# bennyguo/instant-nsr-pl

Measured on NVIDIA H100. Metric: rays/sec fwd+bwd (NeRF-Synthetic lego shape), higher is better.
Workload: dtype f16

## Files before the change

### instant-nsr-pl_b200/csrc/nerf_fused_bwd.cu

```cuda
#include "nerf_fused.cuh"
#include "wgmma.cuh"

namespace {

constexpr int kWarps = 4;
constexpr int kThreads = kWarps * 32;
constexpr int kRows = kWarps * 16;
constexpr int kCtasPerSm = 2;

constexpr int T_X0 = 0;
constexpr int T_H1 = T_X0 + kRows * NF_LD32;
constexpr int T_CI = T_H1 + kRows * NSR_LD64;
constexpr int T_G1 = T_CI + kRows * NF_LD32;
constexpr int T_G2 = T_G1 + kRows * NSR_LD64;
constexpr int T_DC3 = T_G2 + kRows * NSR_LD64;
constexpr int T_DG2 = T_DC3 + kRows * 24;
constexpr int T_DG1 = T_DG2 + kRows * NSR_LD64;
constexpr int T_DO = T_DG1 + kRows * NSR_LD64;
constexpr int T_DH1 = T_DO + kRows * 24;
constexpr int T_X0B = T_DH1 + kRows * NSR_LD64;
constexpr int T_TOTAL = T_X0B + kRows * NF_LD32;
constexpr int S_XYZ = 0, S_DS = S_XYZ + kRows * 6, S_DRGB = S_DS + kRows, S_ROWF = S_DRGB + kRows * 3;
constexpr size_t kSmemBytes = (size_t)(NF_W_TOTAL + T_TOTAL) * sizeof(__half) + 2 * S_ROWF * sizeof(float);
constexpr size_t kSmemBytesVanilla = kSmemBytes + NF_B_TOTAL * sizeof(float);
// ... 191 lines not shown
            for (int e = 0; e < 2; ++e) {
              const int col = c * 2 + e;
              if (col < 3) {
                const float raw = NET == NF_NET_VANILLA ? acc16[0][0][hh * 2 + e] : __half2float(__float2half_rn(acc16[0][0][hh * 2 + e]));
                const float s = 1.f / (1.f + expf(-raw));
                const float dr = PACKED ? rf[S_DRGB + (r0 + g + hh * 8) * 3 + col] : d_rgb[pi * 3 + col];
                dp[hh * 2 + e] = dr * s * (1.f - s) * loss_scale;
              }
            }
          }
        }
      }
      a_dc3[0][0][0] = nsr_pack_h2(dp[0], dp[1]);
      a_dc3[0][0][1] = nsr_pack_h2(dp[2], dp[3]);
      a_dc3[0][0][2] = 0u;
      a_dc3[0][0][3] = 0u;
      nsr_store_afrag<1, 1>(a_dc3, T + T_DC3, 24, r0);
    }
    uint32_t a_d[1][4][4];
    nsr_zero_acc(acc);
    nsr_gemm_wt<1, 1, 8>(acc, a_dc3, smem + NF_OFF_CW3, NSR_LD64);
    relu_mask_pack(acc, a_g2, a_d);
    nsr_store_afrag<1, 4>(a_d, T + T_DG2, NSR_LD64, r0);
    nsr_zero_acc(acc);
    nsr_gemm_wt<1, 4, 8>(acc, a_d, smem + NF_OFF_CW2, NSR_LD64);
    relu_mask_pack(acc, a_g1, a_d);
    nsr_store_afrag<1, 4>(a_d, T + T_DG1, NSR_LD64, r0);
    nsr_zero_acc(acc16);
    nsr_gemm_wt<1, 4, 2>(acc16, a_d, smem + NF_OFF_CW1, NF_LD32);
    if (c == 0) {
      if (ia < n) acc16[0][0][0] += (PACKED ? rf[S_DS + r0 + g] : d_sraw[pa]) * loss_scale;
      if (ib < n) acc16[0][0][2] += (PACKED ? rf[S_DS + r0 + g + 8] : d_sraw[pb]) * loss_scale;
    }
    uint32_t a_do[1][1][4];
    nsr_acc_to_afrag<1, 2>(acc16, a_do, NSR_ACT_NONE);
    nsr_store_afrag<1, 1>(a_do, T + T_DO, 24, r0);
    nsr_zero_acc(acc);
    nsr_gemm_wt<1, 1, 8>(acc, a_do, smem + NF_OFF_DW2, NSR_LD64);
    relu_mask_pack(acc, a_h1, a_d);
    nsr_store_afrag<1, 4>(a_d, T + T_DH1, NSR_LD64, r0);
    float accE[1][4][4];
    nsr_zero_acc(accE);
    nsr_gemm_wt<1, 4, 4>(accE, a_d, smem + NF_OFF_DW1, NF_LD32);

#pragma unroll
    for (int hh = 0; hh < 2; ++hh) {
      const int64_t i = hh ? ib : ia;
      const bool ok = i < n;
      float x = 0.f, y = 0.f, z = 0.f, dx, dy, dz;
      if (ok) {
        if (PACKED) {
          const float* rr = rf + S_XYZ + (r0 + g + hh * 8) * 6;
          x = rr[0];
          y = rr[1];
          z = rr[2];
        } else {
          nf_sample_position<CT>(P, rays, ray_indices[i], t_starts[i], t_ends[i], x, y, z, dx, dy, dz);
        }
      }
#pragma unroll
      for (int nt = 0; nt < 4; ++nt) {
        const float d0 = ok ? accE[0][nt][hh * 2] * inv_scale : 0.f, d1 = ok ? accE[0][nt][hh * 2 + 1] * inv_scale : 0.f;
        const LevelInfo li = nsr_level(P.grid, nt * 4 + c);
        uint32_t cx, cy, cz, idx[8];
        float fx, fy, fz;
        nsr_pos_fract(x, li.scale, cx, fx);
        nsr_pos_fract(y, li.scale, cy, fy);
        nsr_pos_fract(z, li.scale, cz, fz);
        if (nt < 2) {
          const uint32_t key = ok ? (cx + li.res * (cy + li.res * cz)) : (0xFFFFFFF0u + g);
          const uint32_t key_prev = __shfl_up_sync(0xffffffffu, key, 4);
          const bool head = (g == 0) || (key_prev != key);
          const int next_head = __shfl_down_sync(0xffffffffu, (int)head, 4);
          const bool tail = (g == 7) || next_head;
          float v[16];
#pragma unroll
          for (int cc = 0; cc < 8; ++cc) {
            const float w = nsr_corner_weight(cc, fx, fy, fz);
            v[2 * cc] = w * d0;
            v[2 * cc + 1] = w * d1;
          }
          bool flag = head;
#pragma unroll
          for (int o = 1; o < 8; o <<= 1) {
            const int f_up = __shfl_up_sync(0xffffffffu, (int)flag, 4 * o);
            const bool take = (g >= o) && !flag;
#pragma unroll
            for (int e = 0; e < 16; ++e) {
              const float u = __shfl_up_sync(0xffffffffu, v[e], 4 * o);
              if (take) v[e] += u;
            }
            if (take) flag = f_up;
          }
          if (ok && tail) {
            nsr_corner_indices(li, cx, cy, cz, idx);
#pragma unroll
            for (int cc = 0; cc < 8; ++cc)
              if (v[2 * cc] != 0.f || v[2 * cc + 1] != 0.f) nsr_red_add_f32x2(grad_table + 2 * (size_t)idx[cc], v[2 * cc], v[2 * cc + 1]);
          }
        } else if (ok && (d0 != 0.f || d1 != 0.f)) {
          nsr_corner_indices(li, cx, cy, cz, idx);
#pragma unroll
          for (int cc = 0; cc < 8; ++cc) {
            const float w = nsr_corner_weight(cc, fx, fy, fz);
            nsr_red_add_f32x2(grad_table + 2 * (size_t)idx[cc], w * d0, w * d1);
          }
        }
      }
    }
    __syncthreads();
#pragma unroll
    for (int s = 0; s < kSlots; ++s) {
      const WgradTile w = wgrad_tile(warp + s * kWarps);
      const int xo = (w.x_off == T_X0) ? x0_off : w.x_off;
      nsr_wgrad_tile(wacc[s][0], wacc[s][1], T + w.dy_off, w.ldy, w.m0, T + xo, w.ldx, w.n0, kRows);
    }
    if (NET == NF_NET_VANILLA) {
#pragma unroll
      for (int q = 0; q < 2; ++q) {
        const int j = threadIdx.x + q * kThreads;
        if (j < NF_B_TOTAL) {
          const __half* col = j < NF_B_D2 ? T + T_DH1 + j : j < NF_B_C1 ? T + T_DO + (j - NF_B_D2) : j < NF_B_C2 ? T + T_DG1 + (j - NF_B_C1)
                                                                                      : j < NF_B_C3 ? T + T_DG2 + (j - NF_B_C2) : T + T_DC3 + (j - NF_B_C3);
          const int ld = (j >= NF_B_D2 && j < NF_B_C1) || j >= NF_B_C3 ? 24 : NSR_LD64;
          float sum = 0.f;
#pragma unroll 8
          for (int r = 0; r < kRows; ++r) sum += __half2float(col[r * ld]);
          bsum[q] += sum;
        }
      }
    }
  }
  if (NET == NF_NET_VANILLA) {
#pragma unroll
    for (int q = 0; q < 2; ++q) {
      const int j = threadIdx.x + q * kThreads;
      if (j < NF_B_TOTAL && bsum[q] != 0.f) atomicAdd(j < NF_B_C1 ? grad_dbias + j : grad_cbias + (j - NF_B_C1), bsum[q] * inv_scale);
    }
  }
#pragma unroll
  for (int s = 0; s < kSlots; ++s) {
    const WgradTile w = wgrad_tile(warp + s * kWarps);
    float* dst = (w.net == 0 ? grad_dparams : grad_cparams) + w.base;
#pragma unroll
    for (int j = 0; j < 2; ++j)
#pragma unroll
      for (int i = 0; i < 4; ++i) {
        const int o = w.m0 + g + ((i >> 1) << 3), ii = w.n0 + j * 8 + c * 2 + (i & 1);
        atomicAdd(dst + (size_t)o * w.in_dim + ii, wacc[s][j][i] * inv_scale);
      }
  }
}

constexpr int kNetThreads = 384;
constexpr int SL_X0 = 0;
constexpr int SL_CI = SL_X0 + kRows * 32 * 2;
constexpr int SL_H1 = SL_CI + kRows * 32 * 2;
constexpr int SL_G1 = SL_H1 + kRows * 64 * 2;
constexpr int SL_G2 = SL_G1 + kRows * 64 * 2;
constexpr int SL_DC3 = SL_G2 + kRows * 64 * 2;
constexpr int SL_DO = SL_DC3 + kRows * 16 * 2;
constexpr int SL_DG2 = SL_DO + kRows * 16 * 2;
constexpr int SL_DG1 = SL_DG2 + kRows * 64 * 2;
constexpr int SL_DH1 = SL_DG1 + kRows * 64 * 2;
constexpr int kSlotBytes = SL_DH1 + kRows * 64 * 2;
constexpr int kNetSlots = 3;
constexpr int N_SLOTS = NF_W_TOTAL * 2;
constexpr int N_STAGE = N_SLOTS + kNetSlots * kSlotBytes;
constexpr int kStageBytes = kRows * NF_LD32 * 2 + S_ROWF * 4;
constexpr int N_BARS = N_STAGE + 2 * kStageBytes;
constexpr size_t kNetSmemBytes = N_BARS + 2 * kNetSlots * 8;
static_assert(N_SLOTS % 128 == 0 && kSlotBytes % 128 == 0 && kStageBytes % 16 == 0 && N_BARS % 8 == 0, "alignment");
static_assert(kNetSmemBytes <= 227 * 1024, "shared memory");

template <int KT>
__device__ __forceinline__ void canon_load_afrag(uint32_t (&a)[1][KT][4], const uint8_t* tile, int K, int row0, int col0 = 0) {
  const int lane = threadIdx.x & 31, mi = lane >> 3, r = lane & 7;
#pragma unroll
  for (int k = 0; k < KT; ++k) nsr_ldmatrix_x4(a[0][k], tile + nsr_canon_off(row0 + (mi & 1) * 8 + r, col0 + k * 16 + (mi >> 1) * 8, K));
}
template <int KT>
__device__ __forceinline__ void canon_store_afrag(const uint32_t (&a)[1][KT][4], uint8_t* tile, int K, int row0, int col0 = 0) {
  const int lane = threadIdx.x & 31, g = lane >> 2, c = lane & 3;
#pragma unroll
  for (int k = 0; k < KT; ++k) {
    const int col = col0 + k * 16 + c * 2;
    *reinterpret_cast<uint32_t*>(tile + nsr_canon_off(row0 + g, col, K)) = a[0][k][0];
    *reinterpret_cast<uint32_t*>(tile + nsr_canon_off(row0 + g + 8, col, K)) = a[0][k][1];
    *reinterpret_cast<uint32_t*>(tile + nsr_canon_off(row0 + g, col + 8, K)) = a[0][k][2];
    *reinterpret_cast<uint32_t*>(tile + nsr_canon_off(row0 + g + 8, col + 8, K)) = a[0][k][3];
  }
}
__device__ __forceinline__ void group_bar(int grp) { asm volatile("bar.sync %0, 128;" ::"r"(1 + grp) : "memory"); }

template <int R>
__device__ __forceinline__ void net_flush(const float (&w)[R], float* dst, int stride_m, int stride_n, float inv_scale) {
  const int lane = threadIdx.x & 31, m0 = 16 * ((threadIdx.x >> 5) & 3) + (lane >> 2), c0 = 2 * (lane & 3);
#pragma unroll
  for (int r = 0; r < R; ++r) {
    const int j = r >> 2, h = (r >> 1) & 1, e = r & 1;
    atomicAdd(dst + (size_t)(m0 + 8 * h) * stride_m + (size_t)(8 * j + c0 + e) * stride_n, w[r] * inv_scale);
  }
}

__global__ void __launch_bounds__(kNetThreads, 1) nerf_bwd_net_kernel(const __half* __restrict__ enc_save, const __half* __restrict__ dparams,
                                                                      const __half* __restrict__ cparams, const float* __restrict__ d_sraw,
                                                                      const float* __restrict__ d_rgb, float* __restrict__ grad_dparams,
                                                                      float* __restrict__ grad_cparams, float loss_scale,
                                                                      const float* __restrict__ amax_ptr, int64_t n_cap,
                                                                      const int64_t* __restrict__ n_dev, const float* __restrict__ xyzdir,
                                                                      uint32_t* __restrict__ denc_out) {
  const int64_t n = n_dev ? min(*n_dev, n_cap) : n_cap;
  extern __shared__ __align__(128) uint8_t smem_net[];
  __half* W = reinterpret_cast<__half*>(smem_net);
  const int warp = threadIdx.x >> 5, lane = threadIdx.x & 31;
  if (loss_scale <= 0.f) {
    const float amax = fmaxf(__ldg(amax_ptr), 1e-30f);
    loss_scale = exp2f(fminf(fmaxf(floorf(log2f(256.f / amax)), -24.f), 60.f));
  }
  const float inv_scale = 1.f / loss_scale;
  const uint32_t sbase = nsr_smem_u32(smem_net);
  auto full_bar = [&](int s) { return sbase + N_BARS + 8u * (uint32_t)s; };
  auto empty_bar = [&](int s) { return sbase + N_BARS + 8u * (uint32_t)(kNetSlots + s); };
  if (threadIdx.x == 0) {
    for (int s = 0; s < kNetSlots; ++s) {
      mbar_init(full_bar(s), 128);
      mbar_init(empty_bar(s), 128);
    }
    asm volatile("fence.mbarrier_init.release.cluster;" ::: "memory");
  }
  nf_stage_weights(W, dparams, cparams, true);
  __syncthreads();
  const int64_t n_tiles = (n + kRows - 1) / kRows;
  const int64_t my_tiles = n_tiles > (int64_t)blockIdx.x ? (n_tiles - 1 - blockIdx.x) / gridDim.x + 1 : 0;

  if (warp < 8) {
    const int grp = warp >> 2, gtid = threadIdx.x & 127, g = lane >> 2, c = lane & 3;
    const int r0 = (warp & 3) * 16;
    __half* sx = reinterpret_cast<__half*>(smem_net + N_STAGE + grp * kStageBytes);
    float* rf = reinterpret_cast<float*>(smem_net + N_STAGE + grp * kStageBytes + kRows * NF_LD32 * 2);
    auto fetch_tile = [&](int64_t it) {
      const int64_t row0 = ((int64_t)blockIdx.x + it * gridDim.x) * kRows;
      for (int v = gtid; v < kRows * 4; v += 128) cp_async16(sx + (v >> 2) * NF_LD32 + (v & 3) * 8, enc_save + (row0 + (v >> 2)) * 32 + (v & 3) * 8);
      if (gtid < kRows * 6 / 4) cp_async16(rf + S_XYZ + gtid * 4, xyzdir + row0 * 6 + gtid * 4);
      if (gtid < kRows / 4) cp_async16(rf + S_DS + gtid * 4, d_sraw + row0 + gtid * 4);
      if (gtid >= 64 && gtid < 64 + kRows * 3 / 4) cp_async16(rf + S_DRGB + (gtid - 64) * 4, d_rgb + row0 * 3 + (gtid - 64) * 4);
      cp_async_commit();
    };
    if (grp < my_tiles) fetch_tile(grp);
    for (int64_t it = grp; it < my_tiles; it += 2) {
      const int s = (int)(it % kNetSlots);
      const int64_t row0 = ((int64_t)blockIdx.x + it * gridDim.x) * kRows;
      cp_async_wait_all();
      group_bar(grp);
      if (row0 + kRows > n) {
        for (int v = gtid; v < kRows * 4; v += 128)
          if (row0 + (v >> 2) >= n) *reinterpret_cast<uint4*>(sx + (v >> 2) * NF_LD32 + (v & 3) * 8) = make_uint4(0, 0, 0, 0);
        for (int v = gtid; v < S_ROWF; v += 128) {
          const int r = v < S_DS ? v / 6 : (v < S_DRGB ? v - S_DS : (v - S_DRGB) / 3);
          if (row0 + r >= n) rf[v] = 0.f;
        }
        group_bar(grp);
      }
      if (it >= kNetSlots) mbar_wait(empty_bar(s), (uint32_t)((it / kNetSlots - 1) & 1), nullptr, 0);
      uint8_t* slot = smem_net + N_SLOTS + s * kSlotBytes;
      const int64_t ia = row0 + r0 + g, ib = ia + 8;
      uint32_t a_in[1][2][4];
      nsr_load_afrag<1, 2>(a_in, sx, NF_LD32, r0);
      canon_store_afrag<2>(a_in, slot + SL_X0, 32, r0);
      if (lane < 16) {
        uint4 s0 = make_uint4(0, 0, 0, 0), s1 = s0;
        if (row0 + r0 + lane < n) {
          float sh[16];
          const float* rr = rf + S_XYZ + (r0 + lane) * 6;
          nsr_sh4(rr[3], rr[4], rr[5], sh);
          s0 = make_uint4(nsr_pack_h2(sh[0], sh[1]), nsr_pack_h2(sh[2], sh[3]), nsr_pack_h2(sh[4], sh[5]), nsr_pack_h2(sh[6], sh[7]));
          s1 = make_uint4(nsr_pack_h2(sh[8], sh[9]), nsr_pack_h2(sh[10], sh[11]), nsr_pack_h2(sh[12], sh[13]), nsr_pack_h2(sh[14], sh[15]));
        }
        *reinterpret_cast<uint4*>(slot + SL_CI + nsr_canon_off(r0 + lane, 16, 32)) = s0;
        *reinterpret_cast<uint4*>(slot + SL_CI + nsr_canon_off(r0 + lane, 24, 32)) = s1;
      }
      float drgb[2][2], dsr[2];
#pragma unroll
      for (int hh = 0; hh < 2; ++hh) {
#pragma unroll
        for (int e = 0; e < 2; ++e) drgb[hh][e] = (c * 2 + e < 3) ? rf[S_DRGB + (r0 + g + hh * 8) * 3 + c * 2 + e] : 0.f;
        dsr[hh] = rf[S_DS + r0 + g + hh * 8];
      }
      group_bar(grp);
      if (it + 2 < my_tiles) fetch_tile(it + 2);

      uint32_t a_h1[1][4][4], a_o[1][1][4], a_g1[1][4][4], a_g2[1][4][4];
      float acc[1][8][4], acc16[1][2][4];
      nsr_zero_acc(acc);
      nsr_gemm_w<1, 2, 8>(acc, a_in, W + NF_OFF_DW1, NF_LD32);
      nsr_acc_to_afrag<1, 8>(acc, a_h1, NSR_ACT_RELU);
      canon_store_afrag<4>(a_h1, slot + SL_H1, 64, r0);
      nsr_zero_acc(acc16);
      nsr_gemm_w<1, 4, 2>(acc16, a_h1, W + NF_OFF_DW2, NSR_LD64);
      nsr_acc_to_afrag<1, 2>(acc16, a_o, NSR_ACT_NONE);
      canon_store_afrag<1>(a_o, slot + SL_CI, 32, r0);
      __syncwarp();
      {
        uint32_t a_c[1][2][4], a_sh[1][1][4];
        canon_load_afrag<1>(a_sh, slot + SL_CI, 32, r0, 16);
#pragma unroll
        for (int j = 0; j < 4; ++j) {
          a_c[0][0][j] = a_o[0][0][j];
          a_c[0][1][j] = a_sh[0][0][j];
        }
        nsr_zero_acc(acc);
        nsr_gemm_w<1, 2, 8>(acc, a_c, W + NF_OFF_CW1, NF_LD32);
      }
      nsr_acc_to_afrag<1, 8>(acc, a_g1, NSR_ACT_RELU);
      canon_store_afrag<4>(a_g1, slot + SL_G1, 64, r0);
      nsr_zero_acc(acc);
      nsr_gemm_w<1, 4, 8>(acc, a_g1, W + NF_OFF_CW2, NSR_LD64);
      nsr_acc_to_afrag<1, 8>(acc, a_g2, NSR_ACT_RELU);
      canon_store_afrag<4>(a_g2, slot + SL_G2, 64, r0);
      nsr_zero_acc(acc16);
      nsr_gemm_w<1, 4, 2>(acc16, a_g2, W + NF_OFF_CW3, NSR_LD64);
      uint32_t a_dc3[1][1][4];
      {
        float dp[4] = {0.f, 0.f, 0.f, 0.f};
        if (c < 2) {
#pragma unroll
          for (int hh = 0; hh < 2; ++hh) {
            if ((hh ? ib : ia) < n) {
#pragma unroll
              for (int e = 0; e < 2; ++e) {
                if (c * 2 + e < 3) {
                  const float raw = __half2float(__float2half_rn(acc16[0][0][hh * 2 + e]));
                  const float sg = 1.f / (1.f + expf(-raw));
                  dp[hh * 2 + e] = drgb[hh][e] * sg * (1.f - sg) * loss_scale;
                }
              }
            }
          }
        }
        a_dc3[0][0][0] = nsr_pack_h2(dp[0], dp[1]);
        a_dc3[0][0][1] = nsr_pack_h2(dp[2], dp[3]);
        a_dc3[0][0][2] = 0u;
        a_dc3[0][0][3] = 0u;
        canon_store_afrag<1>(a_dc3, slot + SL_DC3, 16, r0);
      }
      uint32_t a_d[1][4][4];
      nsr_zero_acc(acc);
      nsr_gemm_wt<1, 1, 8>(acc, a_dc3, W + NF_OFF_CW3, NSR_LD64);
      relu_mask_pack(acc, a_g2, a_d);
      canon_store_afrag<4>(a_d, slot + SL_DG2, 64, r0);
      nsr_zero_acc(acc);
      nsr_gemm_wt<1, 4, 8>(acc, a_d, W + NF_OFF_CW2, NSR_LD64);
      relu_mask_pack(acc, a_g1, a_d);
      canon_store_afrag<4>(a_d, slot + SL_DG1, 64, r0);
      nsr_zero_acc(acc16);
      nsr_gemm_wt<1, 4, 2>(acc16, a_d, W + NF_OFF_CW1, NF_LD32);
      if (c == 0) {
        if (ia < n) acc16[0][0][0] += dsr[0] * loss_scale;
        if (ib < n) acc16[0][0][2] += dsr[1] * loss_scale;
      }
      uint32_t a_do[1][1][4];
      nsr_acc_to_afrag<1, 2>(acc16, a_do, NSR_ACT_NONE);
      canon_store_afrag<1>(a_do, slot + SL_DO, 16, r0);
      nsr_zero_acc(acc);
      nsr_gemm_wt<1, 1, 8>(acc, a_do, W + NF_OFF_DW2, NSR_LD64);
      relu_mask_pack(acc, a_h1, a_d);
      canon_store_afrag<4>(a_d, slot + SL_DH1, 64, r0);
      nsr_proxy_fence();
      mbar_arrive(full_bar(s));
      float accE[1][4][4];
      nsr_zero_acc(accE);
      nsr_gemm_wt<1, 4, 4>(accE, a_d, W + NF_OFF_DW1, NF_LD32);
#pragma unroll
      for (int hh = 0; hh < 2; ++hh) {
        const int64_t i = hh ? ib : ia;
        if (i < n) {
#pragma unroll
          for (int nt = 0; nt < 4; ++nt) denc_out[i * 16 + nt * 4 + c] = nsr_pack_h2(accE[0][nt][hh * 2], accE[0][nt][hh * 2 + 1]);
        }
      }
    }
  } else {
    float w_dw1[16], w_dw2t[8], w_cw1[16], w_cw2[32], w_cw3t[8];
#pragma unroll
    for (int i = 0; i < 32; ++i) {
      if (i < 8) w_dw2t[i] = w_cw3t[i] = 0.f;
      if (i < 16) w_dw1[i] = w_cw1[i] = 0.f;
      w_cw2[i] = 0.f;
    }
    for (int64_t it = 0; it < my_tiles; ++it) {
      const int s = (int)(it % kNetSlots);
      mbar_wait(full_bar(s), (uint32_t)((it / kNetSlots) & 1), nullptr, 0);
      const uint32_t sl = sbase + N_SLOTS + (uint32_t)s * kSlotBytes;
      nsr_wg_fence();
#pragma unroll
      for (int kk = 0; kk < 4; ++kk) {
        nsr_wgmma_n32<1, 1>(w_dw1, nsr_wg_desc_mn(sl + SL_DH1, 64, kk), nsr_wg_desc_mn(sl + SL_X0, 32, kk), 1u);
        nsr_wgmma_n16<1, 1>(w_dw2t, nsr_wg_desc_mn(sl + SL_H1, 64, kk), nsr_wg_desc_mn(sl + SL_DO, 16, kk), 1u);
        nsr_wgmma_n32<1, 1>(w_cw1, nsr_wg_desc_mn(sl + SL_DG1, 64, kk), nsr_wg_desc_mn(sl + SL_CI, 32, kk), 1u);
        nsr_wgmma_n64<1, 1>(w_cw2, nsr_wg_desc_mn(sl + SL_DG2, 64, kk), nsr_wg_desc_mn(sl + SL_G1, 64, kk), 1u);
        nsr_wgmma_n16<1, 1>(w_cw3t, nsr_wg_desc_mn(sl + SL_G2, 64, kk), nsr_wg_desc_mn(sl + SL_DC3, 16, kk), 1u);
      }
      nsr_wg_commit();
      nsr_wg_wait0();
      nsr_wg_fence_regs(w_dw1);
      nsr_wg_fence_regs(w_dw2t);
      nsr_wg_fence_regs(w_cw1);
      nsr_wg_fence_regs(w_cw2);
      nsr_wg_fence_regs(w_cw3t);
      mbar_arrive(empty_bar(s));
    }
    if (my_tiles > 0) {
      net_flush(w_dw1, grad_dparams, 32, 1, inv_scale);
      net_flush(w_dw2t, grad_dparams + 64 * 32, 1, 64, inv_scale);
      net_flush(w_cw1, grad_cparams, 32, 1, inv_scale);
      net_flush(w_cw2, grad_cparams + 64 * 32, 64, 1, inv_scale);
      net_flush(w_cw3t, grad_cparams + 64 * 32 + 64 * 64, 1, 64, inv_scale);
    }
  }
}

}

namespace {

constexpr int kMergeLevels = 8;

__global__ void __launch_bounds__(256, 5) nerf_table_scatter_kernel(const __grid_constant__ nsr_grid_t g, const float* __restrict__ xyz, int stride,
                                                                 const __half2* __restrict__ denc, float loss_scale,
                                                                 const float* __restrict__ amax_ptr, float* __restrict__ grad_table,
                                                                 int64_t n_cap, const int64_t* __restrict__ n_dev, int l_begin, int l_end) {
  const int64_t n = n_dev ? min(*n_dev, n_cap) : n_cap;
  if (loss_scale <= 0.f) {
    const float amax = fmaxf(__ldg(amax_ptr), 1e-30f);
    loss_scale = exp2f(fminf(fmaxf(floorf(log2f(256.f / amax)), -24.f), 60.f));
  }
  const float inv_scale = 1.f / loss_scale;
  const int lane = threadIdx.x & 31;
  const int64_t n32 = (n + 31) & ~31ll;
  for (int64_t i = blockIdx.x * 256ll + threadIdx.x; i < n32; i += (int64_t)gridDim.x * 256) {
    const bool ok = i < n;
    float x = 0.f, y = 0.f, z = 0.f;
    if (ok) {
      x = xyz[i * stride];
      y = xyz[i * stride + 1];
      z = xyz[i * stride + 2];
    }
    uint2 dq = make_uint2(0u, 0u);
#pragma unroll 1
    for (int l = l_begin; l < l_end; ++l) {
      float2 d = make_float2(0.f, 0.f);
      if (ok) {
        if (l == l_begin || (l & 1) == 0) dq = __ldg(reinterpret_cast<const uint2*>(denc + i * 16 + (l & ~1)));
        const uint32_t h = (l & 1) ? dq.y : dq.x;
        d = __half22float2(*reinterpret_cast<const __half2*>(&h));
        d.x *= inv_scale;
        d.y *= inv_scale;
      }
      const LevelInfo li = nsr_level(g, l);
      uint32_t cx, cy, cz, idx[8];
      float fx, fy, fz;
      nsr_pos_fract(x, li.scale, cx, fx);
      nsr_pos_fract(y, li.scale, cy, fy);
      nsr_pos_fract(z, li.scale, cz, fz);
      float v[16];
#pragma unroll
      for (int c = 0; c < 8; ++c) {
        const float w = nsr_corner_weight(c, fx, fy, fz);
        v[2 * c] = w * d.x;
        v[2 * c + 1] = w * d.y;
      }
      bool issue = ok && (d.x != 0.f || d.y != 0.f);
      if (l < kMergeLevels) {
        const uint32_t key = ok ? (cx + li.res * (cy + li.res * cz)) : (0xFFFFFF00u + lane);
        const uint32_t prev = __shfl_up_sync(0xffffffffu, key, 1);
        const bool head = lane == 0 || prev != key;
        const uint32_t heads = __ballot_sync(0xffffffffu, head);
        const int my_head = 31 - __clz(heads & (0xffffffffu >> (31 - lane)));
        const bool tail = lane == 31 || ((heads >> (lane + 1)) & 1u);
        int maxrun = lane - my_head + 1;
#pragma unroll
        for (int o = 16; o > 0; o >>= 1) maxrun = max(maxrun, __shfl_xor_sync(0xffffffffu, maxrun, o));
#pragma unroll
        for (int o = 1; o < 32; o <<= 1) {
          if (o < maxrun) {
            const bool take = lane - o >= my_head;
#pragma unroll
            for (int e = 0; e < 16; ++e) {
              const float u = __shfl_up_sync(0xffffffffu, v[e], o);
              if (take) v[e] += u;
            }
          }
        }
        issue = ok && tail;
      }
      if (issue) {
        nsr_corner_indices(li, cx, cy, cz, idx);
#pragma unroll
        for (int c = 0; c < 8; c += 2) nsr_red_corner_pair(grad_table, idx[c], idx[c + 1], v[2 * c], v[2 * c + 1], v[2 * c + 2], v[2 * c + 3]);
      }
    }
  }
}

int field_bwd_launch(const nsr_nerf_t* f, const float* rays, const int32_t* ray_indices, const float* t_starts, const float* t_ends,
                     const void* enc_save_h, const void* dparams_h, const void* cparams_h, const float* d_sraw, const float* d_rgb,
                     float* grad_dparams, float* grad_cparams, float loss_scale, const float* amax, int64_t k, const int64_t* k_dev,
                     const int64_t* row_pos, const float* xyzdir, void* stream, const char* who) {
  NSR_REQUIRE(f != nullptr, "%s: field descriptor is NULL", who);
  NSR_REQUIRE(f->grid.n_levels == 16 && f->grid.n_features == 2 && f->feature_dim == 16 && f->density_hidden == 1 && f->color_hidden == 2,
              "%s: fused path needs L=16, F=2, feature_dim=16, hidden layers 1/2", who);
  NSR_REQUIRE(loss_scale > 0.f || amax != nullptr, "%s: loss_scale <= 0 (automatic) needs the amax pointer", who);
  if (k == 0) return 0;
  NSR_REQUIRE(xyzdir == nullptr || row_pos == nullptr, "%s: packed inputs (xyzdir) and row_pos are mutually exclusive", who);
  NSR_REQUIRE(f->contraction == NF_AABB || (f->contraction == NF_UNBOUNDED_SPHERE && xyzdir == nullptr),
              "%s: contraction type %d not implemented here (AABB=0; UN_BOUNDED_SPHERE=2 only without xyzdir)", who, f->contraction);
  static thread_local bool attr_set = false;
  if (!attr_set) {
    cudaError_t e = cudaFuncSetAttribute(nerf_bwd_kernel<false, NF_AABB, NF_NET_FULLY_FUSED>, cudaFuncAttributeMaxDynamicSharedMemorySize, (int)kSmemBytes);
    if (e == cudaSuccess)
      e = cudaFuncSetAttribute(nerf_bwd_kernel<true, NF_AABB, NF_NET_FULLY_FUSED>, cudaFuncAttributeMaxDynamicSharedMemorySize, (int)kSmemBytes);
    if (e == cudaSuccess)
      e = cudaFuncSetAttribute(nerf_bwd_kernel<false, NF_UNBOUNDED_SPHERE, NF_NET_FULLY_FUSED>, cudaFuncAttributeMaxDynamicSharedMemorySize,
                               (int)kSmemBytes);
    if (e != cudaSuccess) {
// ... 142 lines not shown
```

### instant-nsr-pl_b200/csrc/wgmma.cuh

```cuda
#pragma once
#include <stdint.h>

__device__ __forceinline__ uint32_t nsr_smem_u32(const void* p) { return (uint32_t)__cvta_generic_to_shared(p); }

__device__ __forceinline__ int nsr_canon_off(int row, int k, int K) { return ((row >> 3) * (K >> 3) + (k >> 3)) * 128 + (row & 7) * 16 + (k & 7) * 2; }

__device__ __forceinline__ uint64_t nsr_wg_desc(uint32_t saddr, uint32_t lbo_bytes, uint32_t sbo_bytes) {
  return (uint64_t)((saddr & 0x3FFFF) >> 4) | ((uint64_t)((lbo_bytes >> 4) & 0x3FFF) << 16) | ((uint64_t)((sbo_bytes >> 4) & 0x3FFF) << 32);
}

__device__ __forceinline__ uint64_t nsr_wg_desc_mn(uint32_t addr, int C, int kk) {
  return nsr_wg_desc(addr + 2u * (uint32_t)(C / 8) * 128u * (uint32_t)kk, (uint32_t)(C / 8) * 128u, 128u);
}

__device__ __forceinline__ void nsr_wg_fence() { asm volatile("wgmma.fence.sync.aligned;" ::: "memory"); }
__device__ __forceinline__ void nsr_wg_commit() { asm volatile("wgmma.commit_group.sync.aligned;" ::: "memory"); }
__device__ __forceinline__ void nsr_wg_wait0() { asm volatile("wgmma.wait_group.sync.aligned 0;" ::: "memory"); }
__device__ __forceinline__ void nsr_proxy_fence() { asm volatile("fence.proxy.async.shared::cta;" ::: "memory"); }

__device__ __forceinline__ void mbar_init(uint32_t bar, uint32_t count) { asm volatile("mbarrier.init.shared::cta.b64 [%0], %1;" ::"r"(bar), "r"(count) : "memory"); }
__device__ __forceinline__ void mbar_arrive(uint32_t bar) { asm volatile("mbarrier.arrive.shared::cta.b64 _, [%0];" ::"r"(bar) : "memory"); }
__device__ __forceinline__ void mbar_wait(uint32_t bar, uint32_t parity, int* status, int code) {
  const long long t0 = clock64();
  for (;;) {
    uint32_t ok;
    asm volatile(
        "{\n\t"
        ".reg .pred p;\n\t"
        "mbarrier.try_wait.parity.shared::cta.b64 p, [%1], %2;\n\t"
        "selp.u32 %0, 1, 0, p;\n\t"
        "}\n"
        : "=r"(ok)
        : "r"(bar), "r"(parity)
        : "memory");
    if (ok) return;
    if (clock64() - t0 > 4000000000ll) {
      if (status) atomicExch(status, code);
      __trap();
    }
  }
}

template <int R>
__device__ __forceinline__ void nsr_wg_fence_regs(float (&d)[R]) {
#pragma unroll
  for (int i = 0; i < R; ++i) asm volatile("" : "+f"(d[i])::"memory");
}

template <int TA, int TB>
__device__ __forceinline__ void nsr_wgmma_n16(float (&d)[8], uint64_t da, uint64_t db, uint32_t accumulate) {
  asm volatile(
      "{\n\t"
      ".reg .pred p;\n\t"
      "setp.ne.b32 p, %10, 0;\n\t"
      "wgmma.mma_async.sync.aligned.m64n16k16.f32.f16.f16 {%0, %1, %2, %3, %4, %5, %6, %7}, %8, %9, p, 1, 1, %11, %12;\n\t"
      "}\n"
      : "+f"(d[0]), "+f"(d[1]), "+f"(d[2]), "+f"(d[3]), "+f"(d[4]), "+f"(d[5]), "+f"(d[6]), "+f"(d[7])
      : "l"(da), "l"(db), "r"(accumulate), "n"(TA), "n"(TB)
      : "memory");
}

template <int TA, int TB>
__device__ __forceinline__ void nsr_wgmma_n32(float (&d)[16], uint64_t da, uint64_t db, uint32_t accumulate) {
  asm volatile(
      "{\n\t"
      ".reg .pred p;\n\t"
      "setp.ne.b32 p, %18, 0;\n\t"
      "wgmma.mma_async.sync.aligned.m64n32k16.f32.f16.f16 {%0, %1, %2, %3, %4, %5, %6, %7, %8, %9, %10, %11, %12, %13, %14, %15}, %16, %17, p, 1, 1, %19, %20;\n\t"
      "}\n"
      : "+f"(d[0]), "+f"(d[1]), "+f"(d[2]), "+f"(d[3]), "+f"(d[4]), "+f"(d[5]), "+f"(d[6]), "+f"(d[7]), "+f"(d[8]), "+f"(d[9]), "+f"(d[10]),
        "+f"(d[11]), "+f"(d[12]), "+f"(d[13]), "+f"(d[14]), "+f"(d[15])
      : "l"(da), "l"(db), "r"(accumulate), "n"(TA), "n"(TB)
      : "memory");
}

template <int TA, int TB>
__device__ __forceinline__ void nsr_wgmma_n64(float (&d)[32], uint64_t da, uint64_t db, uint32_t accumulate) {
  asm volatile(
      "{\n\t"
      ".reg .pred p;\n\t"
      "setp.ne.b32 p, %34, 0;\n\t"
      "wgmma.mma_async.sync.aligned.m64n64k16.f32.f16.f16 {%0, %1, %2, %3, %4, %5, %6, %7, %8, %9, %10, %11, %12, %13, %14, %15, %16, %17, "
      "%18, %19, %20, %21, %22, %23, %24, %25, %26, %27, %28, %29, %30, %31}, %32, %33, p, 1, 1, %35, %36;\n\t"
      "}\n"
      : "+f"(d[0]), "+f"(d[1]), "+f"(d[2]), "+f"(d[3]), "+f"(d[4]), "+f"(d[5]), "+f"(d[6]), "+f"(d[7]), "+f"(d[8]), "+f"(d[9]), "+f"(d[10]),
        "+f"(d[11]), "+f"(d[12]), "+f"(d[13]), "+f"(d[14]), "+f"(d[15]), "+f"(d[16]), "+f"(d[17]), "+f"(d[18]), "+f"(d[19]), "+f"(d[20]),
        "+f"(d[21]), "+f"(d[22]), "+f"(d[23]), "+f"(d[24]), "+f"(d[25]), "+f"(d[26]), "+f"(d[27]), "+f"(d[28]), "+f"(d[29]), "+f"(d[30]),
        "+f"(d[31])
      : "l"(da), "l"(db), "r"(accumulate), "n"(TA), "n"(TB)
      : "memory");
}

template <int N, int TA, int TB>
__device__ __forceinline__ void nsr_wgmma(float (&d)[N / 2], uint64_t da, uint64_t db, uint32_t accumulate) {
  if constexpr (N == 16) nsr_wgmma_n16<TA, TB>(d, da, db, accumulate);
  else if constexpr (N == 32) nsr_wgmma_n32<TA, TB>(d, da, db, accumulate);
  else nsr_wgmma_n64<TA, TB>(d, da, db, accumulate);
}
```

Baseline: 14.77 million.

## Use register-A wgmma for backward net chain and add third chain group

Replaces the per-warp mma.sync GEMMs in the backward net kernel's per-tile MLP chain with warpgroup wgmma that takes its A operand from registers and reads weights from shared memory staged in canonical layout. It also raises the number of 128-thread chain groups from two to three, each with its own input staging buffer, so more tiles run at once. The aim is higher tensor-core throughput and more latency hiding. In exchange there is a commit and wait after every small GEMM, more threads sharing the SM, and extra shared memory.

```diff
diff --git a/instant-nsr-pl_b200/csrc/nerf_fused_bwd.cu b/instant-nsr-pl_b200/csrc/nerf_fused_bwd.cu
--- a/instant-nsr-pl_b200/csrc/nerf_fused_bwd.cu
+++ b/instant-nsr-pl_b200/csrc/nerf_fused_bwd.cu
@@ -367,7 +367,8 @@
   }
 }
 
-constexpr int kNetThreads = 384;
+constexpr int kChainGroups = 3;
+constexpr int kNetThreads = (kChainGroups + 1) * 128;
 constexpr int SL_X0 = 0;
 constexpr int SL_CI = SL_X0 + kRows * 32 * 2;
 constexpr int SL_H1 = SL_CI + kRows * 32 * 2;
@@ -380,10 +381,15 @@
 constexpr int SL_DH1 = SL_DG1 + kRows * 64 * 2;
 constexpr int kSlotBytes = SL_DH1 + kRows * 64 * 2;
 constexpr int kNetSlots = 3;
-constexpr int N_SLOTS = NF_W_TOTAL * 2;
+constexpr int NW_DW1 = 0;
+constexpr int NW_DW2 = NW_DW1 + 64 * 32 * 2;
+constexpr int NW_CW1 = NW_DW2 + 16 * 64 * 2;
+constexpr int NW_CW2 = NW_CW1 + 64 * 32 * 2;
+constexpr int NW_CW3 = NW_CW2 + 64 * 64 * 2;
+constexpr int N_SLOTS = NW_CW3 + 16 * 64 * 2;
 constexpr int N_STAGE = N_SLOTS + kNetSlots * kSlotBytes;
 constexpr int kStageBytes = kRows * NF_LD32 * 2 + S_ROWF * 4;
-constexpr int N_BARS = N_STAGE + 2 * kStageBytes;
+constexpr int N_BARS = N_STAGE + kChainGroups * kStageBytes;
 constexpr size_t kNetSmemBytes = N_BARS + 2 * kNetSlots * 8;
 static_assert(N_SLOTS % 128 == 0 && kSlotBytes % 128 == 0 && kStageBytes % 16 == 0 && N_BARS % 8 == 0, "alignment");
 static_assert(kNetSmemBytes <= 227 * 1024, "shared memory");
@@ -407,6 +413,33 @@
   }
 }
 __device__ __forceinline__ void group_bar(int grp) { asm volatile("bar.sync %0, 128;" ::"r"(1 + grp) : "memory"); }
+
+__device__ __forceinline__ void canon_stage(uint8_t* dst, const __half* __restrict__ src, int rows, int K) {
+  const int vec_per_row = K / 8;
+  for (int i = threadIdx.x; i < rows * vec_per_row; i += blockDim.x) {
+    const int r = i / vec_per_row, kc = i % vec_per_row;
+    *reinterpret_cast<uint4*>(dst + nsr_canon_off(r, kc * 8, K)) = __ldg(reinterpret_cast<const uint4*>(src + (size_t)r * K) + kc);
+  }
+}
+
+template <int N, int KT, int TB>
+__device__ __forceinline__ void chain_gemm(float (&acc)[1][N / 8][4], const uint32_t (&a)[1][KT][4], uint32_t w, int ldw) {
+  float(&d)[N / 2] = *reinterpret_cast<float(*)[N / 2]>(&acc[0][0][0]);
+#pragma unroll
+  for (int kk = 0; kk < KT; ++kk)
+#pragma unroll
+    for (int i = 0; i < 4; ++i) asm volatile("" ::"r"(a[0][kk][i]) : "memory");
+  nsr_wg_fence_regs(d);
+  nsr_wg_fence();
+#pragma unroll
+  for (int kk = 0; kk < KT; ++kk) {
+    const uint64_t db = TB ? nsr_wg_desc_mn(w, ldw, kk) : nsr_wg_desc(w + 256u * (uint32_t)kk, 128u, (uint32_t)(ldw / 8) * 128u);
+    nsr_wgmma_rs<N, TB>(d, a[0][kk], db, kk > 0 ? 1u : 0u);
+  }
+  nsr_wg_commit();
+  nsr_wg_wait0();
+  nsr_wg_fence_regs(d);
+}
 
 template <int R>
 __device__ __forceinline__ void net_flush(const float (&w)[R], float* dst, int stride_m, int stride_n, float inv_scale) {
@@ -427,7 +460,6 @@
                                                                       uint32_t* __restrict__ denc_out) {
   const int64_t n = n_dev ? min(*n_dev, n_cap) : n_cap;
   extern __shared__ __align__(128) uint8_t smem_net[];
-  __half* W = reinterpret_cast<__half*>(smem_net);
   const int warp = threadIdx.x >> 5, lane = threadIdx.x & 31;
   if (loss_scale <= 0.f) {
     const float amax = fmaxf(__ldg(amax_ptr), 1e-30f);
@@ -444,12 +476,17 @@
     }
     asm volatile("fence.mbarrier_init.release.cluster;" ::: "memory");
   }
-  nf_stage_weights(W, dparams, cparams, true);
+  canon_stage(smem_net + NW_DW1, dparams, 64, 32);
+  canon_stage(smem_net + NW_DW2, dparams + 64 * 32, 16, 64);
+  canon_stage(smem_net + NW_CW1, cparams, 64, 32);
+  canon_stage(smem_net + NW_CW2, cparams + 64 * 32, 64, 64);
+  canon_stage(smem_net + NW_CW3, cparams + 64 * 32 + 64 * 64, 16, 64);
+  nsr_proxy_fence();
   __syncthreads();
   const int64_t n_tiles = (n + kRows - 1) / kRows;
   const int64_t my_tiles = n_tiles > (int64_t)blockIdx.x ? (n_tiles - 1 - blockIdx.x) / gridDim.x + 1 : 0;
 
-  if (warp < 8) {
+  if (warp < 4 * kChainGroups) {
     const int grp = warp >> 2, gtid = threadIdx.x & 127, g = lane >> 2, c = lane & 3;
     const int r0 = (warp & 3) * 16;
     __half* sx = reinterpret_cast<__half*>(smem_net + N_STAGE + grp * kStageBytes);
@@ -463,7 +500,7 @@
       cp_async_commit();
     };
     if (grp < my_tiles) fetch_tile(grp);
-    for (int64_t it = grp; it < my_tiles; it += 2) {
+    for (int64_t it = grp; it < my_tiles; it += kChainGroups) {
       const int s = (int)(it % kNetSlots);
       const int64_t row0 = ((int64_t)blockIdx.x + it * gridDim.x) * kRows;
       cp_async_wait_all();
@@ -503,16 +540,14 @@
         dsr[hh] = rf[S_DS + r0 + g + hh * 8];
       }
       group_bar(grp);
-      if (it + 2 < my_tiles) fetch_tile(it + 2);
+      if (it + kChainGroups < my_tiles) fetch_tile(it + kChainGroups);
 
       uint32_t a_h1[1][4][4], a_o[1][1][4], a_g1[1][4][4], a_g2[1][4][4];
       float acc[1][8][4], acc16[1][2][4];
-      nsr_zero_acc(acc);
-      nsr_gemm_w<1, 2, 8>(acc, a_in, W + NF_OFF_DW1, NF_LD32);
+      chain_gemm<64, 2, 0>(acc, a_in, sbase + NW_DW1, 32);
       nsr_acc_to_afrag<1, 8>(acc, a_h1, NSR_ACT_RELU);
       canon_store_afrag<4>(a_h1, slot + SL_H1, 64, r0);
-      nsr_zero_acc(acc16);
-      nsr_gemm_w<1, 4, 2>(acc16, a_h1, W + NF_OFF_DW2, NSR_LD64);
+      chain_gemm<16, 4, 0>(acc16, a_h1, sbase + NW_DW2, 64);
       nsr_acc_to_afrag<1, 2>(acc16, a_o, NSR_ACT_NONE);
       canon_store_afrag<1>(a_o, slot + SL_CI, 32, r0);
       __syncwarp();
@@ -524,17 +559,14 @@
           a_c[0][0][j] = a_o[0][0][j];
           a_c[0][1][j] = a_sh[0][0][j];
         }
-        nsr_zero_acc(acc);
-        nsr_gemm_w<1, 2, 8>(acc, a_c, W + NF_OFF_CW1, NF_LD32);
+        chain_gemm<64, 2, 0>(acc, a_c, sbase + NW_CW1, 32);
       }
       nsr_acc_to_afrag<1, 8>(acc, a_g1, NSR_ACT_RELU);
       canon_store_afrag<4>(a_g1, slot + SL_G1, 64, r0);
-      nsr_zero_acc(acc);
-      nsr_gemm_w<1, 4, 8>(acc, a_g1, W + NF_OFF_CW2, NSR_LD64);
+      chain_gemm<64, 4, 0>(acc, a_g1, sbase + NW_CW2, 64);
       nsr_acc_to_afrag<1, 8>(acc, a_g2, NSR_ACT_RELU);
       canon_store_afrag<4>(a_g2, slot + SL_G2, 64, r0);
-      nsr_zero_acc(acc16);
-      nsr_gemm_w<1, 4, 2>(acc16, a_g2, W + NF_OFF_CW3, NSR_LD64);
+      chain_gemm<16, 4, 0>(acc16, a_g2, sbase + NW_CW3, 64);
       uint32_t a_dc3[1][1][4];
       {
         float dp[4] = {0.f, 0.f, 0.f, 0.f};
@@ -560,16 +592,13 @@
         canon_store_afrag<1>(a_dc3, slot + SL_DC3, 16, r0);
       }
       uint32_t a_d[1][4][4];
-      nsr_zero_acc(acc);
-      nsr_gemm_wt<1, 1, 8>(acc, a_dc3, W + NF_OFF_CW3, NSR_LD64);
+      chain_gemm<64, 1, 1>(acc, a_dc3, sbase + NW_CW3, 64);
       relu_mask_pack(acc, a_g2, a_d);
       canon_store_afrag<4>(a_d, slot + SL_DG2, 64, r0);
-      nsr_zero_acc(acc);
-      nsr_gemm_wt<1, 4, 8>(acc, a_d, W + NF_OFF_CW2, NSR_LD64);
+      chain_gemm<64, 4, 1>(acc, a_d, sbase + NW_CW2, 64);
       relu_mask_pack(acc, a_g1, a_d);
       canon_store_afrag<4>(a_d, slot + SL_DG1, 64, r0);
-      nsr_zero_acc(acc16);
-      nsr_gemm_wt<1, 4, 2>(acc16, a_d, W + NF_OFF_CW1, NF_LD32);
+      chain_gemm<16, 4, 1>(acc16, a_d, sbase + NW_CW1, 32);
       if (c == 0) {
         if (ia < n) acc16[0][0][0] += dsr[0] * loss_scale;
         if (ib < n) acc16[0][0][2] += dsr[1] * loss_scale;
@@ -577,15 +606,13 @@
       uint32_t a_do[1][1][4];
       nsr_acc_to_afrag<1, 2>(acc16, a_do, NSR_ACT_NONE);
       canon_store_afrag<1>(a_do, slot + SL_DO, 16, r0);
-      nsr_zero_acc(acc);
-      nsr_gemm_wt<1, 1, 8>(acc, a_do, W + NF_OFF_DW2, NSR_LD64);
+      chain_gemm<64, 1, 1>(acc, a_do, sbase + NW_DW2, 64);
       relu_mask_pack(acc, a_h1, a_d);
       canon_store_afrag<4>(a_d, slot + SL_DH1, 64, r0);
       nsr_proxy_fence();
       mbar_arrive(full_bar(s));
       float accE[1][4][4];
-      nsr_zero_acc(accE);
-      nsr_gemm_wt<1, 4, 4>(accE, a_d, W + NF_OFF_DW1, NF_LD32);
+      chain_gemm<32, 4, 1>(accE, a_d, sbase + NW_DW1, 32);
 #pragma unroll
       for (int hh = 0; hh < 2; ++hh) {
         const int64_t i = hh ? ib : ia;
diff --git a/instant-nsr-pl_b200/csrc/wgmma.cuh b/instant-nsr-pl_b200/csrc/wgmma.cuh
--- a/instant-nsr-pl_b200/csrc/wgmma.cuh
+++ b/instant-nsr-pl_b200/csrc/wgmma.cuh
@@ -97,3 +97,55 @@
   else if constexpr (N == 32) nsr_wgmma_n32<TA, TB>(d, da, db, accumulate);
   else nsr_wgmma_n64<TA, TB>(d, da, db, accumulate);
 }
+
+template <int TB>
+__device__ __forceinline__ void nsr_wgmma_rs_n16(float (&d)[8], const uint32_t (&a)[4], uint64_t db, uint32_t accumulate) {
+  asm volatile(
+      "{\n\t"
+      ".reg .pred p;\n\t"
+      "setp.ne.b32 p, %13, 0;\n\t"
+      "wgmma.mma_async.sync.aligned.m64n16k16.f32.f16.f16 {%0, %1, %2, %3, %4, %5, %6, %7}, {%8, %9, %10, %11}, %12, p, 1, 1, %14;\n\t"
+      "}\n"
+      : "+f"(d[0]), "+f"(d[1]), "+f"(d[2]), "+f"(d[3]), "+f"(d[4]), "+f"(d[5]), "+f"(d[6]), "+f"(d[7])
+      : "r"(a[0]), "r"(a[1]), "r"(a[2]), "r"(a[3]), "l"(db), "r"(accumulate), "n"(TB)
+      : "memory");
+}
+
+template <int TB>
+__device__ __forceinline__ void nsr_wgmma_rs_n32(float (&d)[16], const uint32_t (&a)[4], uint64_t db, uint32_t accumulate) {
+  asm volatile(
+      "{\n\t"
+      ".reg .pred p;\n\t"
+      "setp.ne.b32 p, %21, 0;\n\t"
+      "wgmma.mma_async.sync.aligned.m64n32k16.f32.f16.f16 {%0, %1, %2, %3, %4, %5, %6, %7, %8, %9, %10, %11, %12, %13, %14, %15}, "
+      "{%16, %17, %18, %19}, %20, p, 1, 1, %22;\n\t"
+      "}\n"
+      : "+f"(d[0]), "+f"(d[1]), "+f"(d[2]), "+f"(d[3]), "+f"(d[4]), "+f"(d[5]), "+f"(d[6]), "+f"(d[7]), "+f"(d[8]), "+f"(d[9]), "+f"(d[10]),
+        "+f"(d[11]), "+f"(d[12]), "+f"(d[13]), "+f"(d[14]), "+f"(d[15])
+      : "r"(a[0]), "r"(a[1]), "r"(a[2]), "r"(a[3]), "l"(db), "r"(accumulate), "n"(TB)
+      : "memory");
+}
+
+template <int TB>
+__device__ __forceinline__ void nsr_wgmma_rs_n64(float (&d)[32], const uint32_t (&a)[4], uint64_t db, uint32_t accumulate) {
+  asm volatile(
+      "{\n\t"
+      ".reg .pred p;\n\t"
+      "setp.ne.b32 p, %37, 0;\n\t"
+      "wgmma.mma_async.sync.aligned.m64n64k16.f32.f16.f16 {%0, %1, %2, %3, %4, %5, %6, %7, %8, %9, %10, %11, %12, %13, %14, %15, %16, %17, "
+      "%18, %19, %20, %21, %22, %23, %24, %25, %26, %27, %28, %29, %30, %31}, {%32, %33, %34, %35}, %36, p, 1, 1, %38;\n\t"
+      "}\n"
+      : "+f"(d[0]), "+f"(d[1]), "+f"(d[2]), "+f"(d[3]), "+f"(d[4]), "+f"(d[5]), "+f"(d[6]), "+f"(d[7]), "+f"(d[8]), "+f"(d[9]), "+f"(d[10]),
+        "+f"(d[11]), "+f"(d[12]), "+f"(d[13]), "+f"(d[14]), "+f"(d[15]), "+f"(d[16]), "+f"(d[17]), "+f"(d[18]), "+f"(d[19]), "+f"(d[20]),
+        "+f"(d[21]), "+f"(d[22]), "+f"(d[23]), "+f"(d[24]), "+f"(d[25]), "+f"(d[26]), "+f"(d[27]), "+f"(d[28]), "+f"(d[29]), "+f"(d[30]),
+        "+f"(d[31])
+      : "r"(a[0]), "r"(a[1]), "r"(a[2]), "r"(a[3]), "l"(db), "r"(accumulate), "n"(TB)
+      : "memory");
+}
+
+template <int N, int TB>
+__device__ __forceinline__ void nsr_wgmma_rs(float (&d)[N / 2], const uint32_t (&a)[4], uint64_t db, uint32_t accumulate) {
+  if constexpr (N == 16) nsr_wgmma_rs_n16<TB>(d, a, db, accumulate);
+  else if constexpr (N == 32) nsr_wgmma_rs_n32<TB>(d, a, db, accumulate);
+  else nsr_wgmma_rs_n64<TB>(d, a, db, accumulate);
+}
```

Result: faster. 15.22 million (median of 6 runs) (+3.1%).
